# graphdeco-inria/hierarchical-3d-gaussians

Hardware: AMD Instinct MI355X
Metric: fwd+bwd frames/s @1080p, 1M Gaussians (higher is better)
Workload: dtype f32

## Files before the change

hierarchical-3d-gaussians_amd/csrc/render.hip:

```cpp
#include <stdlib.h>

#include "common.h"

namespace hgs {
namespace {

constexpr float kAlphaMin = 1.0f / 255.0f;
constexpr float kAlphaMax = 0.99f;
constexpr float kTEps = 0.0001f;
constexpr float kBig = 1.0e18f;
constexpr int kFwdBatch = 64;
constexpr int kBwdBatch = 64;

struct TileGeom {
  int tile, tx, ty;
};

__device__ __forceinline__ bool block_to_tile(int T, int gx, const uint32_t* __restrict__ order, TileGeom& tg) {
  const int per = (T + 7) >> 3;
  const int b = blockIdx.x;
  const int tile = order ? (int)order[b] : (b & 7) * per + (b >> 3);
  if ((uint32_t)tile >= (uint32_t)T) return false;
  tg.tile = tile;
  tg.ty = tile / gx;
  tg.tx = tile - tg.ty * gx;
  return true;
}

typedef float f2 __attribute__((ext_vector_type(2)));
__device__ __forceinline__ f2 fma2(f2 a, f2 b, f2 c) { return __builtin_elementwise_fma(a, b, c); }
__device__ __forceinline__ f2 splat(float v) { return f2{v, v}; }

__device__ __forceinline__ float exp2_le1(float x) { return __builtin_amdgcn_fmed3f(__builtin_amdgcn_exp2f(x), 0.0f, 1.0f); }

__device__ __forceinline__ const float4* record_at(const float4* lrec, uint32_t off) {
  return reinterpret_cast<const float4*>(reinterpret_cast<const char*>(lrec) + off);
}
__device__ __forceinline__ const float4* entry_record(const float4* lrec, uint32_t e) { return record_at(lrec, e & 0xffffu); }

__device__ __forceinline__ float lod_alpha_remap(float a, float w, float ik, float* d) {
  const float ac = fminf(a, kAlphaMax);
  const float base = 1.0f - ac;
  const float pw = __builtin_amdgcn_exp2f(ik * __builtin_amdgcn_logf(base));
  const bool on = ik > 0.0f;
  if (d) *d = on ? w + (1.0f - w) * (a <= kAlphaMax ? ik * pw * __builtin_amdgcn_rcpf(base) : 0.0f) : 1.0f;
  return on ? w * a + (1.0f - w) * (1.0f - pw) : a;
}

__device__ __forceinline__ void set_priority(int q) {
  if (q >= 3) __builtin_amdgcn_s_setprio(3);
  else if (q == 2) __builtin_amdgcn_s_setprio(2);
  else if (q == 1) __builtin_amdgcn_s_setprio(1);
  else __builtin_amdgcn_s_setprio(0);
}

__device__ __forceinline__ uint32_t rank_below(uint64_t m) {
  return __builtin_amdgcn_mbcnt_hi((uint32_t)(m >> 32), __builtin_amdgcn_mbcnt_lo((uint32_t)m, 0u));
}

struct LaneGeom {
  int q, lx, ly0;
};
__device__ __forceinline__ LaneGeom lane_geom(int lane) {
  LaneGeom g;
  g.q = lane >> 4;
  g.lx = (lane & 7) + ((g.q & 1) << 3);
  g.ly0 = ((lane >> 3) & 1) + ((g.q >> 1) << 3);
  return g;
}

struct QuadHit {
  bool q0, q1, q2, q3;
};
__device__ __forceinline__ float edge_max(float A2, float B2, float C2, float nb2c, float dx, float ly, float hy) {
  const float dy = fminf(fmaxf(nb2c * dx, ly), hy);
  return fmaf(dy, fmaf(C2, dy, B2 * dx), A2 * dx * dx);
}
__device__ __forceinline__ QuadHit quad_hit(float gxt, float gyt, float ex, float ey, float A2, float B2, float C2,
                                            float thr) {
  const bool xl = (gxt - ex <= 7.0f) && (gxt + ex >= 0.0f);
  const bool xr = (gxt - ex <= 15.0f) && (gxt + ex >= 8.0f);
  const bool yt = (gyt - ey <= 7.0f) && (gyt + ey >= 0.0f);
  const bool yb = (gyt - ey <= 15.0f) && (gyt + ey >= 8.0f);
  QuadHit h{xl && yt, xr && yt, xl && yb, xr && yb};
  const float lx[2] = {0.0f - gxt, 8.0f - gxt}, hx[2] = {7.0f - gxt, 15.0f - gxt};
  const float ly[2] = {0.0f - gyt, 8.0f - gyt}, hy[2] = {7.0f - gyt, 15.0f - gyt};
  const float nb2c = -0.5f * B2 * __builtin_amdgcn_rcpf(C2), nb2a = -0.5f * B2 * __builtin_amdgcn_rcpf(A2);
  const float lim = thr - 0.02f;
  bool e[4];
#pragma unroll
  for (int q = 0; q < 4; ++q) {
    const int cx = q & 1, cy = q >> 1;
    const bool in_x = lx[cx] <= 0.0f && hx[cx] >= 0.0f, in_y = ly[cy] <= 0.0f && hy[cy] >= 0.0f;
    const float dxe = lx[cx] > 0.0f ? lx[cx] : hx[cx];
    const float dye = ly[cy] > 0.0f ? ly[cy] : hy[cy];
    const float pv = edge_max(A2, B2, C2, nb2c, dxe, ly[cy], hy[cy]);
    const float ph = edge_max(C2, B2, A2, nb2a, dye, lx[cx], hx[cx]);
    const bool miss_v = in_x || (pv < lim), miss_h = in_y || (ph < lim);
    e[q] = (in_x && in_y) || !(miss_v && miss_h);
  }
  h.q0 = h.q0 && e[0]; h.q1 = h.q1 && e[1]; h.q2 = h.q2 && e[2]; h.q3 = h.q3 && e[3];
  return h;
}

template <bool DEPTH>
struct FwdPair {
  f2 fly, T, Cr, Cg, Cb, Dd;
  uint32_t last0, last1;
};

template <bool DEPTH, bool LODA = false>
__device__ __forceinline__ void fwd_pair_live(FwdPair<DEPTH>& p, f2 pw, const float4& q1,
                                              const float4& q2, uint32_t idx1, float lw = 0.0f, float lik = 0.0f) {
  const f2 G = {exp2_le1(pw.x), exp2_le1(pw.y)};
  f2 araw = q1.y * G;
  if constexpr (LODA) araw = f2{lod_alpha_remap(araw.x, lw, lik, nullptr), lod_alpha_remap(araw.y, lw, lik, nullptr)};
  const f2 alpha = {fminf(kAlphaMax, araw.x), fminf(kAlphaMax, araw.y)};
  const bool live0 = alpha.x >= kAlphaMin;
  const bool live1 = alpha.y >= kAlphaMin;
  const f2 Tn = p.T * (1.0f - alpha);
  const uint64_t l0 = __ballot(live0), l1 = __ballot(live1);
  const uint64_t g0 = __ballot(!(Tn.x < kTEps)), g1 = __ballot(!(Tn.y < kTEps));
  const bool blend0 = __builtin_amdgcn_inverse_ballot_w64(l0 & g0), blend1 = __builtin_amdgcn_inverse_ballot_w64(l1 & g1);
  const bool stop0 = __builtin_amdgcn_inverse_ballot_w64(l0 & ~g0), stop1 = __builtin_amdgcn_inverse_ballot_w64(l1 & ~g1);
  const f2 aT = alpha * p.T;
  const f2 w = {blend0 ? aT.x : 0.0f, blend1 ? aT.y : 0.0f};
  p.Cr = fma2(w, splat(q1.z), p.Cr);
  p.Cg = fma2(w, splat(q1.w), p.Cg);
  p.Cb = fma2(w, splat(q2.x), p.Cb);
  if (DEPTH) p.Dd = fma2(w, splat(q2.y), p.Dd);
  p.T = f2{blend0 ? Tn.x : p.T.x, blend1 ? Tn.y : p.T.y};
  p.last0 = blend0 ? idx1 : p.last0;
  p.last1 = blend1 ? idx1 : p.last1;
  p.fly.x = stop0 ? kBig : p.fly.x;
  p.fly.y = stop1 ? kBig : p.fly.y;
}

template <bool DEPTH, bool LODA>
__global__ __launch_bounds__(64) void render_fwd_quad_kernel(
    const uint32_t* __restrict__ ranges, const uint32_t* __restrict__ point_list,
    const float4* __restrict__ records, int W, int H, int gx, int T, const float* __restrict__ bg,
    float* __restrict__ out_color, float* __restrict__ out_invdepth, float* __restrict__ final_T,
    uint32_t* __restrict__ n_contrib, const uint32_t* __restrict__ order, const float* __restrict__ lod_w,
    const int32_t* __restrict__ lod_kids) {
  constexpr int kB = kFwdBatch;
  constexpr int kLds = LODA ? 4 : 3;
  __shared__ float4 lrec[(kB + 1) * kLds];
  __shared__ uint2 qlist[kB + 3];
  constexpr uint32_t kRecBytes = kLds * 16;

  TileGeom tg;
  if (!block_to_tile(T, gx, order, tg)) return;
  const int lane = threadIdx.x;
  const LaneGeom lg = lane_geom(lane);
  const int px = tg.tx * kTile + lg.lx;
  const int py0 = tg.ty * kTile + lg.ly0;
  const float flx = (float)lg.lx;
  const float tile_x0 = (float)(tg.tx * kTile), tile_y0 = (float)(tg.ty * kTile);

  bool inside[4];
#pragma unroll
  for (int s = 0; s < 4; ++s) inside[s] = (px < W) && (py0 + 2 * s < H);
  FwdPair<DEPTH> P0, P1;
  P0.fly = f2{inside[0] ? (float)lg.ly0 : kBig, inside[1] ? (float)(lg.ly0 + 2) : kBig};
  P1.fly = f2{inside[2] ? (float)(lg.ly0 + 4) : kBig, inside[3] ? (float)(lg.ly0 + 6) : kBig};
  P0.T = P1.T = splat(1.0f);
  P0.Cr = P0.Cg = P0.Cb = P0.Dd = P1.Cr = P1.Cg = P1.Cb = P1.Dd = splat(0.0f);
  P0.last0 = P0.last1 = P1.last0 = P1.last1 = 0;

  const uint32_t r0 = ranges[tg.tile * 2 + 0], r1 = ranges[tg.tile * 2 + 1];
  uint64_t alive = __ballot(inside[0] || inside[1] || inside[2] || inside[3]);
  if (lane == 0) {
    lrec[kB * kLds + 0] = make_float4(0.f, 0.f, 0.f, 0.f);
    lrec[kB * kLds + 1] = make_float4(0.f, 0.f, 0.f, 0.f);
    lrec[kB * kLds + 2] = make_float4(0.f, 0.f, __builtin_inff(), 0.f);
    if constexpr (LODA) lrec[kB * kLds + 3] = make_float4(1.f, 0.f, 0.f, 0.f);
  }
  const uint16_t* myq = reinterpret_cast<const uint16_t*>(qlist) + lg.q;

  for (uint32_t base = r0; base < r1 && alive != 0; base += kB) {
    const uint32_t n = (uint32_t)__builtin_amdgcn_readfirstlane((int)min((uint32_t)kB, r1 - base));
    __syncthreads();
    QuadHit hit{false, false, false, false};
    if ((uint32_t)lane < n) {
      const uint32_t gid = point_list[base + lane];
      const float4* r = records + (size_t)gid * kRecVec;
      float4 a0 = r[0], a2 = r[2];
      const float4 a3 = r[3];
      a0.x = (a0.x - tile_x0) + a3.x;
      a0.y = (a0.y - tile_y0) + a3.y;
      const float4 a1 = r[1];
      hit = quad_hit(a0.x, a0.y, a2.z, a3.w, a0.z, a0.w, a1.x, a3.z);
      a2.z = a3.z;
      lrec[lane * kLds + 0] = a0;
      lrec[lane * kLds + 1] = a1;
      lrec[lane * kLds + 2] = a2;
      if constexpr (LODA) {
        const int kids = lod_kids[gid];
        lrec[lane * kLds + 3] = make_float4(lod_w[gid], kids >= 2 ? 1.0f / (float)kids : 0.0f, 0.f, 0.f);
      }
    }
    hit.q0 = hit.q0 && (alive & 0xffffull) != 0;
    hit.q1 = hit.q1 && (alive & 0xffff0000ull) != 0;
    hit.q2 = hit.q2 && (alive & 0xffff00000000ull) != 0;
    hit.q3 = hit.q3 && (alive & 0xffff000000000000ull) != 0;
    const uint64_t m0 = __ballot(hit.q0), m1 = __ballot(hit.q1), m2 = __ballot(hit.q2), m3 = __ballot(hit.q3);
    for (int i = lane; i < kB + 3; i += 64) qlist[i] = make_uint2(0x00010001u * (kB * kRecBytes), 0x00010001u * (kB * kRecBytes));
    uint16_t* ql16 = reinterpret_cast<uint16_t*>(qlist);
    const uint16_t mine = (uint16_t)((uint32_t)lane * kRecBytes);
    if (hit.q0) ql16[rank_below(m0) * 4 + 0] = mine;
    if (hit.q1) ql16[rank_below(m1) * 4 + 1] = mine;
    if (hit.q2) ql16[rank_below(m2) * 4 + 2] = mine;
    if (hit.q3) ql16[rank_below(m3) * 4 + 3] = mine;
    const int nmax = max(max(__builtin_popcountll(m0), __builtin_popcountll(m1)),
                         max(__builtin_popcountll(m2), __builtin_popcountll(m3)));
    __syncthreads();
    auto visit = [&](uint32_t j, const float4& q0, const float4& q1, const float4& q2) {
      float lw = 0.0f, lik = 0.0f;
      if constexpr (LODA) {
        const float4 q3 = record_at(lrec, j)[3];
        lw = q3.x;
        lik = q3.y;
      }
      const float gyt = q0.y;
      const float dx = q0.x - flx;
      const float ax = q0.z * dx * dx;
      const float bx = q0.w * dx;
      const uint32_t idx1 = (base - r0 + 1) * kRecBytes + j;
      const f2 dy0 = gyt - P0.fly;
      const f2 pw0 = fma2(dy0, fma2(splat(q1.x), dy0, splat(bx)), splat(ax));
      const f2 dy1 = gyt - P1.fly;
      const f2 pw1 = fma2(dy1, fma2(splat(q1.x), dy1, splat(bx)), splat(ax));
      fwd_pair_live<DEPTH, LODA>(P0, pw0, q1, q2, idx1, lw, lik);
      fwd_pair_live<DEPTH, LODA>(P1, pw1, q1, q2, idx1, lw, lik);
    };
    uint32_t jA = myq[0], jB = myq[4];
    float4 A0 = record_at(lrec, jA)[0], A1 = record_at(lrec, jA)[1], A2 = record_at(lrec, jA)[2];
    for (int it = 0; it < nmax; it += 2) {
      const float4 B0 = record_at(lrec, jB)[0], B1 = record_at(lrec, jB)[1], B2 = record_at(lrec, jB)[2];
      const uint32_t jA2 = myq[(it + 2) * 4];
      visit(jA, A0, A1, A2);
      if (it + 1 < nmax) {
        A0 = record_at(lrec, jA2)[0]; A1 = record_at(lrec, jA2)[1]; A2 = record_at(lrec, jA2)[2];
        const uint32_t jB2 = myq[(it + 3) * 4];
        visit(jB, B0, B1, B2);
        jB = jB2;
      }
      jA = jA2;
    }
    alive = __ballot(fminf(fminf(P0.fly.x, P0.fly.y), fminf(P1.fly.x, P1.fly.y)) < kBig);
  }

  const float b0 = bg[0], b1 = bg[1], b2 = bg[2];
  const size_t plane = (size_t)W * H;
  const float Tf[4] = {P0.T.x, P0.T.y, P1.T.x, P1.T.y};
  const float cr[4] = {P0.Cr.x, P0.Cr.y, P1.Cr.x, P1.Cr.y};
  const float cg[4] = {P0.Cg.x, P0.Cg.y, P1.Cg.x, P1.Cg.y};
  const float cb[4] = {P0.Cb.x, P0.Cb.y, P1.Cb.x, P1.Cb.y};
  const float dd[4] = {P0.Dd.x, P0.Dd.y, P1.Dd.x, P1.Dd.y};
  const uint32_t la[4] = {P0.last0 / kRecBytes, P0.last1 / kRecBytes, P1.last0 / kRecBytes, P1.last1 / kRecBytes};
#pragma unroll
  for (int s = 0; s < 4; ++s) {
    if (inside[s]) {
      const size_t pix = (size_t)(py0 + 2 * s) * W + px;
      out_color[pix] = cr[s] + Tf[s] * b0;
      out_color[plane + pix] = cg[s] + Tf[s] * b1;
      out_color[2 * plane + pix] = cb[s] + Tf[s] * b2;
      if (DEPTH) out_invdepth[pix] = dd[s];
      final_T[pix] = Tf[s];
      n_contrib[pix] = la[s];
    }
  }
}

struct BwdPair {
  f2 fly, T, A, bgd, gd;
  f2 c0, c1, c2;
  uint32_t nc0, nc1;
};
struct BwdSums {
  float a0, a1, a4, s6, s7, s8, s9;
};

template <bool DEPTH, bool FIRST, bool LODA = false>
__device__ __forceinline__ void bwd_pair_live(BwdPair& p, BwdSums& S, f2 pw, f2 dy, bool c0, bool c1,
                                              const float4& q1, f2 q2, float lw = 0.0f, float lik = 0.0f) {
  const f2 G = {exp2_le1(pw.x), exp2_le1(pw.y)};
  f2 araw0 = q1.y * G;
  f2 xfac = araw0;
  if constexpr (LODA) {
    float d0, d1;
    const f2 og = araw0;
    araw0 = f2{lod_alpha_remap(og.x, lw, lik, &d0), lod_alpha_remap(og.y, lw, lik, &d1)};
    xfac = f2{og.x * d0, og.y * d1};
  }
  const bool live0 = c0 && (araw0.x >= kAlphaMin);
  const bool live1 = c1 && (araw0.y >= kAlphaMin);
  const f2 araw = {live0 ? araw0.x : 0.0f, live1 ? araw0.y : 0.0f};
  if constexpr (LODA) xfac = f2{live0 ? xfac.x : 0.0f, live1 ? xfac.y : 0.0f};
  const f2 ae = {fminf(kAlphaMax, araw.x), fminf(kAlphaMax, araw.y)};
  const f2 oma = 1.0f - ae;
  const f2 rinv = {__builtin_amdgcn_rcpf(oma.x), __builtin_amdgcn_rcpf(oma.y)};
  const f2 Tcur = p.T * rinv;
  const f2 g0 = p.c0, g1 = p.c1, g2 = p.c2;
  f2 q = fma2(g2, splat(q2.x), fma2(g1, splat(q1.w), g0 * q1.z));
  if (DEPTH) q = fma2(p.gd, splat(q2.y), q);
  const f2 qA = q - p.A;
  const f2 dLda = fma2(qA, Tcur, -(p.bgd * rinv));
  const f2 w = ae * Tcur;
  const f2 X = (LODA ? xfac : araw) * dLda;
  const f2 Xdy = X * dy;
  if (FIRST) {
    S.a0 = X.x + X.y;
    S.a1 = Xdy.x + Xdy.y;
    S.a4 = fmaf(Xdy.y, dy.y, Xdy.x * dy.x);
    S.s6 = fmaf(w.y, g0.y, w.x * g0.x);
    S.s7 = fmaf(w.y, g1.y, w.x * g1.x);
    S.s8 = fmaf(w.y, g2.y, w.x * g2.x);
    if (DEPTH) S.s9 = fmaf(w.y, p.gd.y, w.x * p.gd.x);
  } else {
    S.a0 += X.x + X.y;
    S.a1 += Xdy.x + Xdy.y;
    S.a4 = fmaf(Xdy.y, dy.y, fmaf(Xdy.x, dy.x, S.a4));
    S.s6 = fmaf(w.y, g0.y, fmaf(w.x, g0.x, S.s6));
    S.s7 = fmaf(w.y, g1.y, fmaf(w.x, g1.x, S.s7));
    S.s8 = fmaf(w.y, g2.y, fmaf(w.x, g2.x, S.s8));
    if (DEPTH) S.s9 = fmaf(w.y, p.gd.y, fmaf(w.x, p.gd.x, S.s9));
  }
  p.T = Tcur;
  p.A = fma2(ae, qA, p.A);
}

__device__ __forceinline__ void row_reduce10(float v0, float v1, float v2, float v3, float v4, float v5, float v6,
                                             float v7, float v8, float v9, float& ta, float& tb, float& tc) {
  float r01, r23, r45, r67, r89;
  asm volatile(
      "s_nop 1\n\t"
      "v_add_f32_dpp %3, %8, %8 row_mirror row_mask:0xf bank_mask:0x3\n\t"
      "v_add_f32_dpp %3, %9, %9 row_mirror row_mask:0xf bank_mask:0xc\n\t"
      "v_add_f32_dpp %4, %10, %10 row_mirror row_mask:0xf bank_mask:0x3\n\t"
      "v_add_f32_dpp %4, %11, %11 row_mirror row_mask:0xf bank_mask:0xc\n\t"
      "v_add_f32_dpp %5, %12, %12 row_mirror row_mask:0xf bank_mask:0x3\n\t"
      "v_add_f32_dpp %5, %13, %13 row_mirror row_mask:0xf bank_mask:0xc\n\t"
      "v_add_f32_dpp %6, %14, %14 row_mirror row_mask:0xf bank_mask:0x3\n\t"
      "v_add_f32_dpp %6, %15, %15 row_mirror row_mask:0xf bank_mask:0xc\n\t"
      "v_add_f32_dpp %7, %16, %16 row_mirror row_mask:0xf bank_mask:0x3\n\t"
      "v_add_f32_dpp %7, %17, %17 row_mirror row_mask:0xf bank_mask:0xc\n\t"
      "v_add_f32_dpp %0, %3, %3 row_half_mirror row_mask:0xf bank_mask:0x5\n\t"
      "v_add_f32_dpp %0, %4, %4 row_half_mirror row_mask:0xf bank_mask:0xa\n\t"
      "v_add_f32_dpp %1, %5, %5 row_half_mirror row_mask:0xf bank_mask:0x5\n\t"
      "v_add_f32_dpp %1, %6, %6 row_half_mirror row_mask:0xf bank_mask:0xa\n\t"
      "v_add_f32_dpp %2, %7, %7 row_half_mirror row_mask:0xf bank_mask:0xf\n\t"
      "v_add_f32_dpp %0, %0, %0 quad_perm:[1,0,3,2] row_mask:0xf bank_mask:0xf\n\t"
      "v_add_f32_dpp %1, %1, %1 quad_perm:[1,0,3,2] row_mask:0xf bank_mask:0xf\n\t"
      "v_add_f32_dpp %2, %2, %2 quad_perm:[1,0,3,2] row_mask:0xf bank_mask:0xf\n\t"
      "v_add_f32_dpp %0, %0, %0 quad_perm:[2,3,0,1] row_mask:0xf bank_mask:0xf\n\t"
      "v_add_f32_dpp %1, %1, %1 quad_perm:[2,3,0,1] row_mask:0xf bank_mask:0xf\n\t"
      "v_add_f32_dpp %2, %2, %2 quad_perm:[2,3,0,1] row_mask:0xf bank_mask:0xf"
      : "=&v"(ta), "=&v"(tb), "=&v"(tc), "=&v"(r01), "=&v"(r23), "=&v"(r45), "=&v"(r67), "=&v"(r89)
      : "v"(v0), "v"(v1), "v"(v2), "v"(v3), "v"(v4), "v"(v5), "v"(v6), "v"(v7), "v"(v8), "v"(v9));
}

constexpr int kK7Waves = 4;
template <bool DEPTH, bool LODA>
__global__ __launch_bounds__(64) __attribute__((amdgpu_waves_per_eu(kK7Waves, kK7Waves))) void render_bwd_quad_kernel(
    const uint32_t* __restrict__ ranges, const uint32_t* __restrict__ point_list,
    const float4* __restrict__ records, int W, int H, int gx, int T, const float* __restrict__ bg,
    const float* __restrict__ final_T, const uint32_t* __restrict__ n_contrib,
    const uint32_t* __restrict__ offsets, const float* __restrict__ dL_dcolor,
    const float* __restrict__ dL_dinvdepth, float* __restrict__ inst, const uint32_t* __restrict__ order,
    const float* __restrict__ lod_w, const int32_t* __restrict__ lod_kids, int last_round_waves) {
  constexpr int kB = kBwdBatch;
  constexpr int kLds = LODA ? 4 : 3;
  __shared__ float4 lrec[(kB + 1) * kLds];
  __shared__ uint4 qlist[kB + 3];
  constexpr uint32_t kRecBytes = kLds * 16, kSlotBytes = kInstStride * 4;
  constexpr int kSlots = LODA ? 124 : 128;
  __shared__ __attribute__((aligned(8))) float acc[(kSlots + 1) * kInstStride];

  TileGeom tg;
  if (!block_to_tile(T, gx, order, tg)) return;
  const int lane = threadIdx.x;
  const LaneGeom lg = lane_geom(lane);
  const int px = tg.tx * kTile + lg.lx;
  const int py0 = tg.ty * kTile + lg.ly0;
  const float flx = (float)lg.lx;
  const float tile_x0 = (float)(tg.tx * kTile), tile_y0 = (float)(tg.ty * kTile);
  const size_t plane = (size_t)W * H;
  const float b0 = bg[0], b1 = bg[1], b2 = bg[2];
  const uint32_t r0 = ranges[tg.tile * 2 + 0], r1 = ranges[tg.tile * 2 + 1];
  const uint32_t total = r1 - r0;
  if (total == 0) return;

  float Tr[4], bgd[4], g0[4], g1[4], g2[4], gd[4];
  uint32_t nc[4];
  uint32_t maxnc = 0;
#pragma unroll
  for (int s = 0; s < 4; ++s) {
    const int py = py0 + 2 * s;
    Tr[s] = 1.0f; bgd[s] = 0.f; g0[s] = g1[s] = g2[s] = gd[s] = 0.f; nc[s] = 0;
    if (px < W && py < H) {
      const size_t pix = (size_t)py * W + px;
      g0[s] = dL_dcolor[pix];
      g1[s] = dL_dcolor[plane + pix];
      g2[s] = dL_dcolor[2 * plane + pix];
      if (DEPTH) gd[s] = dL_dinvdepth[pix];
      Tr[s] = final_T[pix];
      bgd[s] = Tr[s] * (g0[s] * b0 + g1[s] * b1 + g2[s] * b2);
      nc[s] = n_contrib[pix];
    }
    maxnc = max(maxnc, nc[s]);
  }
#pragma unroll
  for (int off = 8; off > 0; off >>= 1) maxnc = max(maxnc, (uint32_t)__shfl_xor((int)maxnc, off, 64));
  const uint32_t qnc0 = (uint32_t)__builtin_amdgcn_readlane((int)maxnc, 0), qnc1 = (uint32_t)__builtin_amdgcn_readlane((int)maxnc, 16);
  const uint32_t qnc2 = (uint32_t)__builtin_amdgcn_readlane((int)maxnc, 32), qnc3 = (uint32_t)__builtin_amdgcn_readlane((int)maxnc, 48);
  maxnc = max(max(qnc0, qnc1), max(qnc2, qnc3));
  BwdPair P0, P1;
  const float flyb = (float)lg.ly0;
  P0.T = f2{Tr[0], Tr[1]};     P1.T = f2{Tr[2], Tr[3]};
  P0.bgd = f2{bgd[0], bgd[1]}; P1.bgd = f2{bgd[2], bgd[3]};
  P0.c0 = f2{g0[0], g0[1]}; P0.c1 = f2{g1[0], g1[1]}; P0.c2 = f2{g2[0], g2[1]};
  P1.c0 = f2{g0[2], g0[3]}; P1.c1 = f2{g1[2], g1[3]}; P1.c2 = f2{g2[2], g2[3]};
  P0.gd = f2{gd[0], gd[1]};    P1.gd = f2{gd[2], gd[3]};
  P0.A = P1.A = splat(0.0f);
  P0.nc0 = nc[0]; P0.nc1 = nc[1]; P1.nc0 = nc[2]; P1.nc1 = nc[3];
  if (lane == 0) {
    lrec[kB * kLds + 0] = make_float4(0.f, 0.f, 0.f, 0.f);
    lrec[kB * kLds + 1] = make_float4(0.f, 0.f, 0.f, 0.f);
    lrec[kB * kLds + 2] = make_float4(0.f, 0.f, __builtin_inff(), 0.f);
    if constexpr (LODA) lrec[kB * kLds + 3] = make_float4(1.f, 0.f, 0.f, 0.f);
  }
  const uint32_t* myq = reinterpret_cast<const uint32_t*>(qlist) + lg.q;
  const int quad = (lane >> 2) & 3;
  const bool writer = (lane & 3) == 0;
  const int ka = ((quad & 1) << 1) | (quad >> 1);
  const int kc = 8 + (quad >> 1);
  const bool writer_c = writer && (quad & 1) == 0;

  const bool last_round = (int)blockIdx.x >= (int)gridDim.x - last_round_waves;
  for (int hi = (int)maxnc; hi > 0;) {
    const int bstart = hi - kB;
    set_priority(last_round ? (hi + kB - 1) / kB - 1 : 3);
    __syncthreads();
    QuadHit hit{false, false, false, false};
    uint32_t my_off = 0, my_rect = 0;
    const bool staged_lane = bstart + lane >= 0;
    if (staged_lane) {
      const uint32_t gid = point_list[r0 + (uint32_t)(bstart + lane)];
      const float4* r = records + (size_t)gid * kRecVec;
      float4 a0 = r[0], a2 = r[2];
      const float4 a3 = r[3];
      a0.x = (a0.x - tile_x0) + a3.x;
      a0.y = (a0.y - tile_y0) + a3.y;
      const float4 a1 = r[1];
      const uint32_t rel = (uint32_t)(bstart + lane);
      hit = quad_hit(a0.x, a0.y, a2.z, a3.w, a0.z, a0.w, a1.x, a3.z);
      hit.q0 = hit.q0 && rel < qnc0; hit.q1 = hit.q1 && rel < qnc1;
      hit.q2 = hit.q2 && rel < qnc2; hit.q3 = hit.q3 && rel < qnc3;
      my_off = offsets[gid];
      my_rect = __float_as_uint(a2.w);
      a2.z = a3.z;
      lrec[lane * kLds + 0] = a0;
      lrec[lane * kLds + 1] = a1;
      lrec[lane * kLds + 2] = a2;
      if constexpr (LODA) {
        const int kids = lod_kids[gid];
        lrec[lane * kLds + 3] = make_float4(lod_w[gid], kids >= 2 ? 1.0f / (float)kids : 0.0f, 0.f, 0.f);
      }
    }
    uint64_t m0 = __ballot(hit.q0), m1 = __ballot(hit.q1), m2 = __ballot(hit.q2), m3 = __ballot(hit.q3);
    int c0n = __builtin_popcountll(m0), c1n = __builtin_popcountll(m1);
    int c2n = __builtin_popcountll(m2), c3n = __builtin_popcountll(m3);
    uint32_t k0 = rank_below(m0), k1 = rank_below(m1), k2 = rank_below(m2), k3 = rank_below(m3);
    int first = 0;
    if (c0n + c1n + c2n + c3n > kSlots) {
      const uint32_t from_here = (uint32_t)(c0n + c1n + c2n + c3n) - (k0 + k1 + k2 + k3);
      const uint64_t keep = __ballot(from_here <= (uint32_t)kSlots);
      first = __builtin_ctzll(keep);
      const uint64_t low = ~keep;
      const int d0 = __builtin_popcountll(m0 & low), d1 = __builtin_popcountll(m1 & low);
      const int d2 = __builtin_popcountll(m2 & low), d3 = __builtin_popcountll(m3 & low);
      m0 &= keep; m1 &= keep; m2 &= keep; m3 &= keep;
      c0n -= d0; c1n -= d1; c2n -= d2; c3n -= d3;
      k0 -= (uint32_t)d0; k1 -= (uint32_t)d1; k2 -= (uint32_t)d2; k3 -= (uint32_t)d3;
      const bool kept = lane >= first;
      hit.q0 = hit.q0 && kept; hit.q1 = hit.q1 && kept; hit.q2 = hit.q2 && kept; hit.q3 = hit.q3 && kept;
    }
    const uint32_t slot0 = k0 + k1 + k2 + k3;
    const uint32_t npairs = (uint32_t)hit.q0 + (uint32_t)hit.q1 + (uint32_t)hit.q2 + (uint32_t)hit.q3;
    {
      const uint32_t none = (uint32_t)kB * kRecBytes | ((uint32_t)kSlots * kSlotBytes << 16);
      for (int i = lane; i < kB + 3; i += 64) qlist[i] = make_uint4(none, none, none, none);
    }
    uint32_t* ql32 = reinterpret_cast<uint32_t*>(qlist);
    {
      uint32_t en = (uint32_t)lane * kRecBytes | (slot0 * kSlotBytes << 16);
      if (hit.q0) { ql32[(c0n - 1 - (int)k0) * 4 + 0] = en; en += kSlotBytes << 16; }
      if (hit.q1) { ql32[(c1n - 1 - (int)k1) * 4 + 1] = en; en += kSlotBytes << 16; }
      if (hit.q2) { ql32[(c2n - 1 - (int)k2) * 4 + 2] = en; en += kSlotBytes << 16; }
      if (hit.q3) { ql32[(c3n - 1 - (int)k3) * 4 + 3] = en; }
    }
    const int nmax = max(max(c0n, c1n), max(c2n, c3n));
    __syncthreads();
    const uint32_t bs = (uint32_t)max(bstart + first, 0);
    P0.fly = f2{P0.nc0 > bs ? flyb : kBig, P0.nc1 > bs ? flyb + 2.0f : kBig};
    P1.fly = f2{P1.nc0 > bs ? flyb + 4.0f : kBig, P1.nc1 > bs ? flyb + 6.0f : kBig};
    auto limit = [&](uint32_t nc) { return (uint32_t)min(max((int)nc - bstart, 0), kB + 1) * kRecBytes; };
    const uint32_t lim0 = limit(P0.nc0), lim1 = limit(P0.nc1), lim2 = limit(P1.nc0), lim3 = limit(P1.nc1);

    auto visit = [&](uint32_t e, const float4& q0, const float4& q1, const float4& q2v, auto&& pin_lookahead) {
      const uint32_t jo = e & 0xffffu;
      const float gyt = q0.y;
      const float dx = q0.x - flx;
      const float ax = q0.z * dx * dx;
      const float bx = q0.w * dx;
      const f2 dy0 = gyt - P0.fly;
      const f2 pw0 = fma2(dy0, fma2(splat(q1.x), dy0, splat(bx)), splat(ax));
      const f2 dy1 = gyt - P1.fly;
      const f2 pw1 = fma2(dy1, fma2(splat(q1.x), dy1, splat(bx)), splat(ax));
      const bool c0 = jo < lim0, c1 = jo < lim1;
      const bool c2 = jo < lim2, c3 = jo < lim3;
      const f2 q2 = f2{q2v.x, q2v.y};
      float lw = 0.0f, lik = 0.0f;
      if constexpr (LODA) {
        const float4 q3 = reinterpret_cast<const float4*>(reinterpret_cast<const char*>(lrec) + jo)[3];
        lw = q3.x;
        lik = q3.y;
      }
      BwdSums S;
      if (!DEPTH) S.s9 = 0.0f;
      bwd_pair_live<DEPTH, true, LODA>(P0, S, pw0, dy0, c0, c1, q1, q2, lw, lik);
      bwd_pair_live<DEPTH, false, LODA>(P1, S, pw1, dy1, c2, c3, q1, q2, lw, lik);
      const float s0 = dx * S.a0, s3 = dx * S.a1;
      const float s2 = dx * s0;
      float ta, tb, tc;
      row_reduce10(s0, S.a1, s2, s3, S.a4, S.a0, S.s6, S.s7, S.s8, S.s9, ta, tb, tc);
      pin_lookahead();
      if (writer) {
        float* row = reinterpret_cast<float*>(reinterpret_cast<char*>(acc) + (e >> 16));
        row[ka] = ta;
        row[4 + ka] = tb;
        if (writer_c) row[kc] = tc;
      }
    };
    {
      uint32_t jA = myq[0], jB = myq[4];
      float4 A0 = entry_record(lrec, jA)[0], A1 = entry_record(lrec, jA)[1], A2 = entry_record(lrec, jA)[2];
      asm volatile("" : : "v"(jB), "v"(A0.x), "v"(A0.y), "v"(A0.z), "v"(A0.w), "v"(A1.x), "v"(A1.y), "v"(A1.z), "v"(A1.w), "v"(A2.x),
                   "v"(A2.y));
      for (int it = 0; it < nmax; it += 2) {
        const float4 B0 = entry_record(lrec, jB)[0], B1 = entry_record(lrec, jB)[1], B2 = entry_record(lrec, jB)[2];
        const uint32_t jA2 = myq[(it + 2) * 4];
        visit(jA, A0, A1, A2, [&] {
          asm volatile("" : : "v"(B0.x), "v"(B0.y), "v"(B0.z), "v"(B0.w), "v"(B1.x), "v"(B1.y), "v"(B1.z), "v"(B1.w), "v"(B2.x),
                       "v"(B2.y), "v"(jA2));
        });
        if (it + 1 < nmax) {
          A0 = entry_record(lrec, jA2)[0]; A1 = entry_record(lrec, jA2)[1]; A2 = entry_record(lrec, jA2)[2];
          const uint32_t jB2 = myq[(it + 3) * 4];
          visit(jB, B0, B1, B2, [&] {
            asm volatile("" : : "v"(A0.x), "v"(A0.y), "v"(A0.z), "v"(A0.w), "v"(A1.x), "v"(A1.y), "v"(A1.z), "v"(A1.w), "v"(A2.x),
                         "v"(A2.y), "v"(jB2));
          });
          jB = jB2;
        }
        jA = jA2;
      }
    }
    __syncthreads();
    if (staged_lane && lane >= first) {
      const uint32_t minx = my_rect & 1023u, miny = (my_rect >> 10) & 1023u, rw = my_rect >> 20;
      const uint32_t e = my_off + ((uint32_t)tg.ty - miny) * rw + ((uint32_t)tg.tx - minx);
      f2* dst = reinterpret_cast<f2*>(inst + (size_t)e * kInstStride);
      const f2* row = reinterpret_cast<const f2*>(acc + slot0 * kInstStride);
      f2 sum[kInstStride / 2];
#pragma unroll
      for (int k = 0; k < kInstStride / 2; ++k) sum[k] = npairs > 0 ? row[k] : splat(0.0f);
#pragma unroll
      for (int t = 1; t < 4; ++t) {
        if ((uint32_t)t < npairs) {
#pragma unroll
          for (int k = 0; k < kInstStride / 2; ++k) sum[k] += row[t * (kInstStride / 2) + k];
        }
      }
#pragma unroll
      for (int k = 0; k < kInstStride / 2; ++k) dst[k] = sum[k];
    }
    hi = bstart + first;
  }
  for (int i = (int)maxnc + lane; i < (int)total; i += 64) {
    const uint32_t gid = point_list[r0 + i];
    const uint32_t rb = __float_as_uint(reinterpret_cast<const float*>(records + (size_t)gid * kRecVec + 2)[3]);
    const uint32_t minx = rb & 1023u, miny = (rb >> 10) & 1023u, rw = rb >> 20;
    const uint32_t e = offsets[gid] + ((uint32_t)tg.ty - miny) * rw + ((uint32_t)tg.tx - minx);
    f2* dst = reinterpret_cast<f2*>(inst + (size_t)e * kInstStride);
#pragma unroll
    for (int k = 0; k < kInstStride / 2; ++k) dst[k] = splat(0.0f);
  }
}

}

int launch_render_fwd(const hgs_raster_args& a, const GeomWs& g, const BinWs& b, const ImgWs& im,
                      float* out_color, float* out_invdepth, hipStream_t s) {
  const int gxx = grid_x(a.width), T = gxx * grid_y(a.height);
  const int nblk = ((T + 7) / 8) * 8;
  const bool depth = a.do_depth && out_invdepth;
  const bool loda = a.lod_per_pixel && a.interpolation_weights && a.num_node_kids;
  auto kern = loda ? (depth ? render_fwd_quad_kernel<true, true> : render_fwd_quad_kernel<false, true>)
                   : (depth ? render_fwd_quad_kernel<true, false> : render_fwd_quad_kernel<false, false>);
  hipLaunchKernelGGL(kern, dim3(nblk), dim3(64), 0, s, b.ranges, b.vals_out,
                     reinterpret_cast<const float4*>(g.records), a.width, a.height, gxx, T, a.bg, out_color,
                     out_invdepth, im.final_T, im.n_contrib, b.tile_order, a.interpolation_weights, a.num_node_kids);
  HGS_LAUNCH_CHECK("render_fwd_quad", s, a.debug);
  return HGS_OK;
}

int launch_render_bwd(const hgs_raster_args& a, const GeomWs& g, const BinWs& b, const ImgWs& im,
                      const float* out_color, const float* out_invdepth, const float* dL_dcolor,
                      const float* dL_dinvdepth, float* inst_grads, hipStream_t s) {
  (void)out_color;
  const int gxx = grid_x(a.width), T = gxx * grid_y(a.height);
  const int nblk = ((T + 7) / 8) * 8;
  const bool depth = a.do_depth && out_invdepth && dL_dinvdepth;
  const bool loda = a.lod_per_pixel && a.interpolation_weights && a.num_node_kids;
  auto kern = loda ? (depth ? render_bwd_quad_kernel<true, true> : render_bwd_quad_kernel<false, true>)
                   : (depth ? render_bwd_quad_kernel<true, false> : render_bwd_quad_kernel<false, false>);
  hipLaunchKernelGGL(kern, dim3(nblk), dim3(64), 0, s, b.ranges, b.vals_out,
                     reinterpret_cast<const float4*>(g.records), a.width, a.height, gxx, T, a.bg, im.final_T,
                     im.n_contrib, g.offsets, dL_dcolor, dL_dinvdepth, inst_grads, b.tile_order, a.interpolation_weights,
                     a.num_node_kids, scan_resident_workgroups() * 4 * kK7Waves);
  HGS_LAUNCH_CHECK("render_bwd_quad", s, a.debug);
  return HGS_OK;
}

}
```

Measured before the change: 1429.

## Cull forward-render Gaussians per 4x4 cell instead of per 8x8 quadrant

```diff
diff --git a/hierarchical-3d-gaussians_amd/csrc/render.hip b/hierarchical-3d-gaussians_amd/csrc/render.hip
--- a/hierarchical-3d-gaussians_amd/csrc/render.hip
+++ b/hierarchical-3d-gaussians_amd/csrc/render.hip
@@ -66,6 +66,17 @@
   g.q = lane >> 4;
   g.lx = (lane & 7) + ((g.q & 1) << 3);
   g.ly0 = ((lane >> 3) & 1) + ((g.q >> 1) << 3);
+  return g;
+}
+
+struct CellGeom {
+  int c, lx, ly0;
+};
+__device__ __forceinline__ CellGeom cell_geom(int lane) {
+  CellGeom g;
+  g.c = lane >> 2;
+  g.lx = ((g.c & 3) << 2) + (lane & 3);
+  g.ly0 = (g.c >> 2) << 2;
   return g;
 }
 
@@ -101,6 +112,19 @@
   }
   h.q0 = h.q0 && e[0]; h.q1 = h.q1 && e[1]; h.q2 = h.q2 && e[2]; h.q3 = h.q3 && e[3];
   return h;
+}
+__device__ __forceinline__ uint32_t cell_hit(float gxt, float gyt, float ex, float ey, float A2, float B2, float C2,
+                                             float thr) {
+  const QuadHit h = quad_hit(gxt, gyt, ex, ey, A2, B2, C2, thr);
+  uint32_t xb = 0, yb = 0;
+#pragma unroll
+  for (int i = 0; i < 4; ++i) {
+    xb |= (uint32_t)((gxt - ex <= (float)(4 * i + 3)) && (gxt + ex >= (float)(4 * i))) << i;
+    yb |= (uint32_t)((gyt - ey <= (float)(4 * i + 3)) && (gyt + ey >= (float)(4 * i))) << i;
+  }
+  const uint32_t box = xb * ((yb & 1u) | ((yb & 2u) << 3) | ((yb & 4u) << 6) | ((yb & 8u) << 9));
+  const uint32_t qm = (h.q0 ? 0x0033u : 0u) | (h.q1 ? 0x00ccu : 0u) | (h.q2 ? 0x3300u : 0u) | (h.q3 ? 0xcc00u : 0u);
+  return box & qm;
 }
 
 template <bool DEPTH>
@@ -136,8 +160,9 @@
   p.fly.y = stop1 ? kBig : p.fly.y;
 }
 
+constexpr int kK6Waves = 6;
 template <bool DEPTH, bool LODA>
-__global__ __launch_bounds__(64) void render_fwd_quad_kernel(
+__global__ __launch_bounds__(64) __attribute__((amdgpu_waves_per_eu(kK6Waves, kK6Waves))) void render_fwd_quad_kernel(
     const uint32_t* __restrict__ ranges, const uint32_t* __restrict__ point_list,
     const float4* __restrict__ records, int W, int H, int gx, int T, const float* __restrict__ bg,
     float* __restrict__ out_color, float* __restrict__ out_invdepth, float* __restrict__ final_T,
@@ -146,13 +171,13 @@
   constexpr int kB = kFwdBatch;
   constexpr int kLds = LODA ? 4 : 3;
   __shared__ float4 lrec[(kB + 1) * kLds];
-  __shared__ uint2 qlist[kB + 3];
+  __shared__ uint4 qlist[(kB + 3) * 2];
   constexpr uint32_t kRecBytes = kLds * 16;
 
   TileGeom tg;
   if (!block_to_tile(T, gx, order, tg)) return;
   const int lane = threadIdx.x;
-  const LaneGeom lg = lane_geom(lane);
+  const CellGeom lg = cell_geom(lane);
   const int px = tg.tx * kTile + lg.lx;
   const int py0 = tg.ty * kTile + lg.ly0;
   const float flx = (float)lg.lx;
@@ -160,10 +185,10 @@
 
   bool inside[4];
 #pragma unroll
-  for (int s = 0; s < 4; ++s) inside[s] = (px < W) && (py0 + 2 * s < H);
+  for (int s = 0; s < 4; ++s) inside[s] = (px < W) && (py0 + s < H);
   FwdPair<DEPTH> P0, P1;
-  P0.fly = f2{inside[0] ? (float)lg.ly0 : kBig, inside[1] ? (float)(lg.ly0 + 2) : kBig};
-  P1.fly = f2{inside[2] ? (float)(lg.ly0 + 4) : kBig, inside[3] ? (float)(lg.ly0 + 6) : kBig};
+  P0.fly = f2{inside[0] ? (float)lg.ly0 : kBig, inside[1] ? (float)(lg.ly0 + 1) : kBig};
+  P1.fly = f2{inside[2] ? (float)(lg.ly0 + 2) : kBig, inside[3] ? (float)(lg.ly0 + 3) : kBig};
   P0.T = P1.T = splat(1.0f);
   P0.Cr = P0.Cg = P0.Cb = P0.Dd = P1.Cr = P1.Cg = P1.Cb = P1.Dd = splat(0.0f);
   P0.last0 = P0.last1 = P1.last0 = P1.last1 = 0;
@@ -176,12 +201,12 @@
     lrec[kB * kLds + 2] = make_float4(0.f, 0.f, __builtin_inff(), 0.f);
     if constexpr (LODA) lrec[kB * kLds + 3] = make_float4(1.f, 0.f, 0.f, 0.f);
   }
-  const uint16_t* myq = reinterpret_cast<const uint16_t*>(qlist) + lg.q;
+  const uint16_t* myq = reinterpret_cast<const uint16_t*>(qlist) + lg.c;
 
   for (uint32_t base = r0; base < r1 && alive != 0; base += kB) {
     const uint32_t n = (uint32_t)__builtin_amdgcn_readfirstlane((int)min((uint32_t)kB, r1 - base));
     __syncthreads();
-    QuadHit hit{false, false, false, false};
+    uint32_t hit = 0;
     if ((uint32_t)lane < n) {
       const uint32_t gid = point_list[base + lane];
       const float4* r = records + (size_t)gid * kRecVec;
@@ -190,7 +215,7 @@
       a0.x = (a0.x - tile_x0) + a3.x;
       a0.y = (a0.y - tile_y0) + a3.y;
       const float4 a1 = r[1];
-      hit = quad_hit(a0.x, a0.y, a2.z, a3.w, a0.z, a0.w, a1.x, a3.z);
+      const float ex = a2.z;
       a2.z = a3.z;
       lrec[lane * kLds + 0] = a0;
       lrec[lane * kLds + 1] = a1;
@@ -199,21 +224,21 @@
         const int kids = lod_kids[gid];
         lrec[lane * kLds + 3] = make_float4(lod_w[gid], kids >= 2 ? 1.0f / (float)kids : 0.0f, 0.f, 0.f);
       }
-    }
-    hit.q0 = hit.q0 && (alive & 0xffffull) != 0;
-    hit.q1 = hit.q1 && (alive & 0xffff0000ull) != 0;
-    hit.q2 = hit.q2 && (alive & 0xffff00000000ull) != 0;
-    hit.q3 = hit.q3 && (alive & 0xffff000000000000ull) != 0;
-    const uint64_t m0 = __ballot(hit.q0), m1 = __ballot(hit.q1), m2 = __ballot(hit.q2), m3 = __ballot(hit.q3);
-    for (int i = lane; i < kB + 3; i += 64) qlist[i] = make_uint2(0x00010001u * (kB * kRecBytes), 0x00010001u * (kB * kRecBytes));
+      hit = cell_hit(a0.x, a0.y, ex, a3.w, a0.z, a0.w, a1.x, a3.z);
+    }
+    const uint32_t live_cells = (uint32_t)__ballot(lane < 16 && ((alive >> (4 * (lane & 15))) & 0xfull) != 0);
+    hit &= live_cells;
+    constexpr uint32_t kNone = 0x00010001u * (kB * kRecBytes);
+    for (int i = lane; i < (kB + 3) * 2; i += 64) qlist[i] = make_uint4(kNone, kNone, kNone, kNone);
     uint16_t* ql16 = reinterpret_cast<uint16_t*>(qlist);
     const uint16_t mine = (uint16_t)((uint32_t)lane * kRecBytes);
-    if (hit.q0) ql16[rank_below(m0) * 4 + 0] = mine;
-    if (hit.q1) ql16[rank_below(m1) * 4 + 1] = mine;
-    if (hit.q2) ql16[rank_below(m2) * 4 + 2] = mine;
-    if (hit.q3) ql16[rank_below(m3) * 4 + 3] = mine;
-    const int nmax = max(max(__builtin_popcountll(m0), __builtin_popcountll(m1)),
-                         max(__builtin_popcountll(m2), __builtin_popcountll(m3)));
+    int nmax = 0;
+#pragma unroll
+    for (int c = 0; c < 16; ++c) {
+      const uint64_t m = __ballot((hit >> c) & 1u);
+      if ((hit >> c) & 1u) ql16[rank_below(m) * 16 + c] = mine;
+      nmax = max(nmax, __builtin_popcountll(m));
+    }
     __syncthreads();
     auto visit = [&](uint32_t j, const float4& q0, const float4& q1, const float4& q2) {
       float lw = 0.0f, lik = 0.0f;
@@ -234,15 +259,15 @@
       fwd_pair_live<DEPTH, LODA>(P0, pw0, q1, q2, idx1, lw, lik);
       fwd_pair_live<DEPTH, LODA>(P1, pw1, q1, q2, idx1, lw, lik);
     };
-    uint32_t jA = myq[0], jB = myq[4];
+    uint32_t jA = myq[0], jB = myq[16];
     float4 A0 = record_at(lrec, jA)[0], A1 = record_at(lrec, jA)[1], A2 = record_at(lrec, jA)[2];
     for (int it = 0; it < nmax; it += 2) {
       const float4 B0 = record_at(lrec, jB)[0], B1 = record_at(lrec, jB)[1], B2 = record_at(lrec, jB)[2];
-      const uint32_t jA2 = myq[(it + 2) * 4];
+      const uint32_t jA2 = myq[(it + 2) * 16];
       visit(jA, A0, A1, A2);
       if (it + 1 < nmax) {
         A0 = record_at(lrec, jA2)[0]; A1 = record_at(lrec, jA2)[1]; A2 = record_at(lrec, jA2)[2];
-        const uint32_t jB2 = myq[(it + 3) * 4];
+        const uint32_t jB2 = myq[(it + 3) * 16];
         visit(jB, B0, B1, B2);
         jB = jB2;
       }
@@ -262,7 +287,7 @@
 #pragma unroll
   for (int s = 0; s < 4; ++s) {
     if (inside[s]) {
-      const size_t pix = (size_t)(py0 + 2 * s) * W + px;
+      const size_t pix = (size_t)(py0 + s) * W + px;
       out_color[pix] = cr[s] + Tf[s] * b0;
       out_color[plane + pix] = cg[s] + Tf[s] * b1;
       out_color[2 * plane + pix] = cb[s] + Tf[s] * b2;
```

New measurement: 1487, median of 6. +4.1%, better.
